# danthegoodman1/ObjectKV

Measured on AMD Instinct MI355X. Metric: GiB/s device-resident SST block decode + M rows/s, at 1/2/4/8 MI355X, higher is better.
Workload: dtype u8; 1 GPU; C3: 65536 x 64 KiB blocks, Zipf key 8-256 B / value 0-4096 B, full decode (arenas + SoA); blocks_per_gpu=65536, segment_bytes_per_gpu=4300412312, block_bytes_per_gpu=4294967296, original_bytes_per_gpu=3848907004, rows_per_gpu=1837903, mode=full, parallelism=1 independent segments (no collective)

## Files before the change

### __graft_entry__.py

```python
from __future__ import annotations

import os
import subprocess
import sys

ROOT = os.path.dirname(os.path.abspath(__file__))


def build() -> None:
    env = dict(os.environ, PYTORCH_ROCM_ARCH="gfx950")
    subprocess.run(["make", "-s", "-C", os.path.join(ROOT, "objectkv_amd", "csrc")], check=True,
                   env=env)
    subprocess.run(["make", "-s", "-C", os.path.join(ROOT, "oracle")], check=True)
    if ROOT not in sys.path:
        sys.path.insert(0, ROOT)
    import objectkv_amd
    objectkv_amd.lib()


def smoke() -> None:
    if ROOT not in sys.path:
        sys.path.insert(0, ROOT)
    import numpy as np

    import objectkv_amd as okv
    from oracle import coracle

    for kind, seed, th, bs in ((okv.sst.SYNTH_ZIPF, 3, 57344, 65536),
                               (okv.sst.SYNTH_FIXED, 1, 3584, 4096)):
        w = okv.synth_segment(kind, seed, nblocks=16, threshold=th, block_size=bs)
        seg, descs = w.data(), w.descs()[:16]
        dec = okv.Decoder(0)
        got = dec.decode(seg, descs)
        ref = coracle.decode_soa(seg, coracle.descs_array([tuple(int(x) for x in d)
                                                           for d in descs]))
# ... 29 lines not shown
```

### objectkv_amd/csrc/okv_ctx.hpp

```cpp
#pragma once
#include <hip/hip_runtime.h>

#include <algorithm>
#include <cstdlib>
#include <string>
#include <vector>

#include "okv_kernels.hpp"
#include "okv_sst.h"

namespace okv {
struct EncScratch;
void enc_release(okv_ctx* ctx);
namespace mrg {
struct Scratch;
}
void merge_release(okv_ctx* ctx);
void launch_hash(hipStream_t stream, const uint8_t* seg, uint64_t seg_bytes, const Desc* descs,
                 uint32_t nblk, uint64_t* out);
void launch_zstd_cap(hipStream_t s, const Desc* descs, uint32_t nblk, uint64_t* cap_off);
int zstd_run(okv_ctx* ctx, const uint8_t* seg, uint64_t seg_bytes, const Desc* descs,
             uint32_t nblk, uint64_t* total);
void launch_zstd_desc(hipStream_t s, const Desc* descs, uint32_t nblk, const uint64_t* cap_off,
                      const uint64_t* dec_len, Desc* out);
constexpr uint32_t kZstdLitBytes = 1u << 17;
}

struct okv_ctx {
  int device = 0;
  hipStream_t stream = nullptr;
// ... 7 lines not shown
  uint32_t* d_big = nullptr;
  uint32_t* d_ctr = nullptr;
  uint32_t big_slot = 0;
  size_t cap_blocks = 0;
  bool fused = true;
  uint32_t fused_max = 0;
  bool zstd_one_pass = false;
  bool point = true;
  uint32_t* f_flag = nullptr;
  okv::Prefix* f_agg = nullptr;
  okv::Prefix* f_incl = nullptr;
  unsigned long long* f_ctr = nullptr;
  unsigned long long f_base = 0;
  uint32_t f_epoch = 0;
  bool group = false;
  uint32_t* g_flag = nullptr;
  okv::Prefix* g_agg = nullptr;
  okv::Prefix* g_incl = nullptr;
  size_t g_cap = 0;
  uint32_t g_epoch = 0;
  uint32_t last_path = 0;
  okv_ctx* chain = nullptr;
  std::vector<okv_ctx*> chained_by;
  hipEvent_t p3_done = nullptr;
  bool p3_rec = false;
  size_t f_cap = 0;
  okv::Totals* d_tot = nullptr;
  okv::Totals* h_tot = nullptr;
  unsigned long long* d_span = nullptr;
  unsigned long long* h_span = nullptr;
  okv::SpanHint span_hint;
  bool pieces = false;
  bool stream_lb = false;
  uint64_t small_piece = 0;
  void* d_ptot = nullptr;
  hipStream_t stream2 = nullptr;
  hipEvent_t ev_piece[2] = {nullptr, nullptr};
  okv::Totals* d_tot2 = nullptr;
  uint8_t* d_seg = nullptr;
  size_t cap_seg = 0;
  okv::Desc* d_desc = nullptr;
  size_t cap_desc = 0;
  void* d_out = nullptr;
  size_t cap_out = 0;
  uint64_t* d_hash = nullptr;
  size_t cap_hash = 0;
// ... 95 lines not shown
```

### objectkv_amd/csrc/okv_decode.hip

```cpp
#include <hip/hip_runtime.h>

#include <algorithm>
#include <atomic>
#include <cstdio>
#include <cstdlib>
#include <cstring>
#include <string>
#include <vector>

#include "okv_ctx.hpp"
#include "okv_kernels.hpp"
#include "okv_sst.h"

namespace okv {

__device__ __forceinline__ uint64_t rec_index(uint32_t , uint32_t b, uint32_t r) {
  return uint64_t(b) * kRCap + r;
}
constexpr uint32_t kRecChunk = 16;

__global__ __launch_bounds__(kThreads) void okv_count_kernel(
    const uint8_t* __restrict__ seg, uint64_t seg_bytes, const Desc* __restrict__ descs,
    uint32_t nblk, int comp, BlockCount* __restrict__ cnt, Prefix* __restrict__ lp,
    Prefix* __restrict__ tile_tot, uint32_t* __restrict__ rt_pos, uint16_t* __restrict__ rt_kl,
// ... 5 lines not shown
  __shared__ uint32_t s_pos[kThreads * (kRecChunk + 1)];
  __shared__ __align__(16) uint16_t s_kl[kThreads * kRecChunk];
  __shared__ uint32_t s_rows[kThreads];
  const uint32_t tid = threadIdx.x;
  const uint32_t b = blockIdx.x * kTile + tid;
  uint64_t rows = 0, kb = 0, vb = 0, p = 0;
  int32_t st = OKV_BLK_OK;
  if (blockIdx.x == 0 && tid == 0 && big_zero) *big_zero = 0;
  uint64_t len = 0, orig = 0, off = 0;
  bool walking = false;
  if (b < nblk) {
    const Desc d = descs[b];
    const int32_t pre = pre_status ? pre_status[b] : int32_t(OKV_BLK_OK);
    if (pre != OKV_BLK_OK) {
      st = pre;
    } else if ((st = go_read_status(d, seg_bytes)) != OKV_BLK_OK) {
    } else if (comp == OKV_COMP_ZSTD) {
      st = OKV_BLK_UNSUPPORTED;
    } else {
      len = (comp == OKV_COMP_LZ4) ? 0 : d.block_size;
      orig = go_walk_bound(d.original_size);
      off = d.offset;
      walking = true;
      if (prefetch && orig && len) {
        const uint64_t first = off & ~uint64_t(3);
        const uint64_t last = (off + (orig < len ? orig : len) - 1) & ~uint64_t(3);
        uint32_t v[32];
#pragma unroll
        for (int u = 0; u < 32; ++u) {
          uint64_t a = (off & ~uint64_t(127)) + 128ull * u;
          a = a < first ? first : (a > last ? last : a);
          v[u] = *reinterpret_cast<const uint32_t*>(seg + a);
        }
        uint32_t acc = 0;
#pragma unroll
        for (int u = 0; u < 32; ++u) acc ^= v[u];
        asm volatile("" ::"v"(acc));
      }
    }
  }
  const uint32_t b0 = blockIdx.x * kTile;
  for (uint32_t c = 0; c < uint32_t(kRCap) / kRecChunk; ++c) {
    const uint64_t cap = uint64_t(c + 1) * kRecChunk;
    if (walking) {
      while (p < orig && rows < cap) {
        if (len - p < 6) { st = OKV_BLK_PANIC; break; }
        uint32_t kl, vl;
        header_global(seg, off + p, kl, vl);
        const uint64_t room = len - p - 6;
        if (kl > room || vl > room - kl) {
          st = OKV_BLK_PANIC;
          break;
        }
        const uint32_t slot = uint32_t(rows) & (kRecChunk - 1);
        s_pos[tid * (kRecChunk + 1) + slot] = uint32_t(p);
        s_kl[tid * kRecChunk + slot] = uint16_t(kl);
        rows++;
        kb += kl;
        vb += vl;
        p += 6 + uint64_t(kl) + uint64_t(vl);
      }
      if (st != OKV_BLK_OK) walking = false;
    }
    s_rows[tid] = st == OKV_BLK_OK ? uint32_t(rows) : 0u;
    __syncthreads();
    for (uint32_t q = tid; q < uint32_t(kTile) * 4; q += kThreads) {
      const uint32_t lb = q >> 2, sub = q & 3, slot = c * kRecChunk + sub * 4;
      if (b0 + lb < nblk && slot < s_rows[lb]) {
        const uint32_t* s = &s_pos[lb * (kRecChunk + 1) + sub * 4];
        *reinterpret_cast<uint4*>(rt_pos + rec_index(nblk, b0 + lb, slot)) =
            make_uint4(s[0], s[1], s[2], s[3]);
// ... 147 lines not shown
  const BlockCount* cnt;
  const Prefix* lp;
  const Prefix* tile_pre;
  const uint32_t* rt_pos;
  const uint16_t* rt_kl;
  uint32_t* big_list;
  uint32_t* big_count;
  uint64_t* row_start;
  uint64_t* key_base;
  uint64_t* val_base;
  int32_t* blk_status;
  uint64_t* key_off;
  uint16_t* key_len;
  uint64_t* val_off;
  uint32_t* val_len;
  uint8_t* key_arena;
  uint8_t* val_arena;
  uint64_t row_cap, key_cap, val_cap;
  uint64_t* vsrc;
  uint32_t* vtile;
  uint4* bchunk;
  const Totals* tot;
  uint64_t span_cap;
};

constexpr uint32_t kSwTile = 4096;
__device__ __forceinline__ bool sweep_safe(const Totals& T, uint32_t nbig, uint64_t row_cap,
                                           uint64_t key_cap, uint64_t val_cap) {
  return nbig == 0 && T.rows <= row_cap && T.kb <= key_cap && T.vb <= val_cap;
}

struct BlockBase {
  uint64_t row0, kb0, vb0;
  int32_t st;
};
__device__ __forceinline__ BlockBase block_base_of(const CopyParams& P, const BlockCount& c,
                                                   const Prefix& l, const Prefix& t) {
  BlockBase r;
  r.row0 = t.rows + l.rows;
  r.kb0 = t.kb + l.kb;
  r.vb0 = t.vb + l.vb;
  r.st = c.status;
  if (r.st == OKV_BLK_OK &&
      (r.row0 + c.rows > P.row_cap ||
       (!P.index_only && (r.kb0 + round16(c.kbytes) > P.key_cap ||
                          r.vb0 + round16(c.vbytes) > P.val_cap))))
// ... 213 lines not shown
    default:
      return make_uint4(funnel(y.x, x.w, r), funnel(y.y, y.x, r), funnel(y.z, y.y, r),
                        funnel(y.w, y.z, r));
  }
}

__device__ __noinline__ uint4 tile_chunk_pieces(const uint8_t* seg, uint64_t seg_bytes, uint64_t off,
                                                const uint32_t* pre, const uint32_t* sb,
                                                uint32_t rows, uint32_t r, uint32_t x,
                                                uint32_t lo, uint32_t hi) {
  const uint32_t dend = min(hi, pre[rows]);
  uint4 out = make_uint4(0, 0, 0, 0);
  for (uint32_t d = lo; d < dend; ++r) {
    const uint32_t e = min(dend, pre[r + 1]);
    if (e > d) {
      out = merge_bytes(out, window16(seg, seg_bytes, int64_t(off + sb[r] + x)), int32_t(d - x),
                        int32_t(e - x));
      d = e;
    }
  }
  return out;
}

template <uint32_t kT, uint32_t kNT, bool kXcd, uint32_t kSkip = 0>
__device__ __forceinline__ void tile_pass(const CopyParams& P, uint32_t tpb, uint32_t ntile) {
  constexpr uint32_t kG = kT / 64 + 8;
  constexpr bool kSector = (kSkip & 128) != 0;
  constexpr bool kLineCut = !(kSkip & 64) && !kSector;
  constexpr bool kKeyRound = kSector && !(kSkip & 256);
  constexpr uint32_t kLineExt = (kLineCut || (kSkip & 512)) ? 512 : 0;
  __shared__ TileRows<kT> R;
  __shared__ uint8_t gt[1][kG];
  __shared__ uint4 stage[(kT + kLineExt) / 16 + 4];
  uint32_t L = blockIdx.x;
  if constexpr (kXcd) L = (blockIdx.x & 7u) * (gridDim.x >> 3) + (blockIdx.x >> 3);
  if (L >= ntile) return;
  const uint32_t b = __builtin_amdgcn_readfirstlane(L / tpb);
  const uint32_t t = L - b * tpb;
  const uint32_t tid = threadIdx.x, lane = tid & 63;
  uint32_t rec = 0, kl = 0;
  if (tid < 64) {
    rec = P.rt_pos[rec_index(P.nblk, b, lane)];
    kl = P.rt_kl[rec_index(P.nblk, b, lane)];
  }
  const uint64_t off = P.descs[b].offset;
  const BlockCount c = P.cnt[b];
  const Prefix lpre = P.lp[b], tpre = P.tile_pre[b / kTile];
  asm volatile("" ::"s"(off), "s"(c.rows), "s"(c.kbytes), "s"(c.vbytes), "s"(c.pend),
               "s"(c.status), "s"(lpre.rows), "s"(lpre.kb), "s"(lpre.vb), "s"(tpre.rows),
               "s"(tpre.kb), "s"(tpre.vb));
  const uint64_t row0 = tpre.rows + lpre.rows, kb0 = tpre.kb + lpre.kb, vb0 = tpre.vb + lpre.vb;
  const bool fits = row0 + c.rows <= P.row_cap &&
                    (P.index_only ||
                     (kb0 + round16(c.kbytes) <= P.key_cap && vb0 + round16(c.vbytes) <= P.val_cap));
  const int32_t st = (c.status == OKV_BLK_OK && !fits) ? int32_t(OKV_BLK_CAPACITY) : c.status;
  auto block_outputs = [&]() {
    if (t == 0 && tid == 0) {
      P.row_start[b] = row0;
      if (P.key_base) P.key_base[b] = kb0;
      if (P.val_base) P.val_base[b] = vb0;
      P.blk_status[b] = st;
    }
  };
  const uint64_t pend = c.pend;
  const uint32_t P0 = t * kT;
  if (st != OKV_BLK_OK || c.rows == 0 || c.rows > uint64_t(kRCap) || pend > P.span_cap ||
      pend >= (uint64_t(1) << 32) || P0 >= pend) {
    block_outputs();
    return;
  }
  const uint32_t rows = uint32_t(c.rows), lastr = rows - 1;
  const uint32_t P1 = uint32_t(min<uint64_t>(uint64_t(P0) + kT, pend));
  const bool last_tile = P1 == pend;
  const int64_t A = int64_t((off + P0) & ~uint64_t(15)) - 16;
  const int64_t E = int64_t((off + P1 + 15) & ~uint64_t(15)) + 16 + (last_tile ? 0 : kLineExt);
  const uint32_t np = uint32_t((E - A) >> 4);
  if (!P.index_only && tid >= 64) {
    const int64_t lim = int64_t(round16(P.seg_bytes));
    const uint32_t u = tid - 64;
    for (uint32_t k0 = 0; k0 < np; k0 += kNT - 64) {
      const uint32_t i = k0 + u;
      if (i < np) {
        int64_t a = A + (int64_t(i) << 4);
        if (a < 0 || a + 16 > lim) a = int64_t(off) & ~int64_t(15);
        __builtin_amdgcn_global_load_lds(P.seg + a, OKV_LDS_PTR(stage + k0 + (u & ~63u)), 16,
                                         0, 0);
      }
    }
  }
  if (tid < 64) {
// ... 140 lines not shown
        const bool eb = piece && (e & 15);
        const uint64_t m = __ballot(eb);
        const uint32_t head = (X2 < X3 && (X2 & 15)) ? 1u : 0u;
        const uint32_t idx = head + uint32_t(__builtin_amdgcn_mbcnt_hi(
                                        uint32_t(m >> 32), __builtin_amdgcn_mbcnt_lo(uint32_t(m), 0u)));
        if (eb) R.bnd[idx] = ((e >> 4) << 8) | lane;
        const uint32_t nunit = __builtin_amdgcn_readlane(ui, 63);
        if (lane == 0) {
          if (head) R.bnd[0] = ((X2 >> 4) << 8) | jv;
          R.nbnd = head + uint32_t(__builtin_popcountll(m));
          R.nunit = nunit;
        }
      }
    }
    if (P.index_only && t == 0 && live) {
      const uint64_t g = row0 + lane;
      P.key_len[g] = uint16_t(k);
      P.val_len[g] = v;
      P.key_off[g] = off + ks;
      P.val_off[g] = off + vs;
    }
  }
  if (P.index_only) {
    block_outputs();
    return;
  }
  if (tid >= 64) asm volatile("s_waitcnt vmcnt(0)" ::: "memory");
  __syncthreads();
  if (t == 0 && tid < 64) {
    block_outputs();
    if (!(kSkip & 1) && lane < rows) {
      const uint64_t g = row0 + lane;
      const uint32_t kp = R.pre[0][lane], vp = R.pre[1][lane];
      P.key_len[g] = uint16_t(R.pre[0][lane + 1] - kp);
      P.val_len[g] = R.pre[1][lane + 1] - vp;
      P.key_off[g] = kb0 + kp;
      P.val_off[g] = vb0 + vp;
    }
  }
  const uint32_t kx0 = R.x[0], kx1 = R.x[1], vx0 = R.x[2], vx1 = R.x[3];
  const uint32_t nk = kx1 > kx0 ? ((kx1 + 15) >> 4) - (kx0 >> 4) : 0u;
  const uint32_t sbias = uint32_t(int64_t(off) - A);
  {
    const uint32_t nunit = R.nunit, nbnd = R.nbnd;
    uint8_t* const varena = P.val_arena + vb0;
    for (uint32_t u = tid >> 6; u < ((kSkip & 2) ? 0u : nunit); u += kNT / 64) {
      const uint32_t c0 = __builtin_amdgcn_readfirstlane(R.unit[0][u]);
      const uint32_t sbyte = __builtin_amdgcn_readfirstlane(R.unit[1][u]);
      const uint32_t cnt = __builtin_amdgcn_readfirstlane(R.unit[2][u]);
      if (lane < cnt) {
        const uint32_t line = (sbyte >> 4) + lane;
// ... 1159 lines not shown
  if ((rc = grow(ctx, reinterpret_cast<void**>(&ctx->z_dec), &ctx->z_cap_dec, total + 64)))
    return rc;
  if ((rc = zstd_run(ctx, d_seg, seg_bytes, d_desc, nblk, &total))) return rc;
  launch_zstd_desc(ctx->stream, d_desc, nblk, ctx->z_cap_off, ctx->z_dec_len, ctx->z_desc);
  OKV_HIP(hipGetLastError());
  *w = Work{ctx->z_dec, total + 16, ctx->z_desc, OKV_COMP_NONE, ctx->z_status};
  return OKV_OK;
}

uint32_t gather_threads(const okv_ctx* ctx, const Work& w, uint32_t nblk) {
  if (ctx->gather_threads) return ctx->gather_threads;
  return nblk && w.seg_bytes / nblk <= 16384 ? 64u : 256u;
}

int launch_plan(okv_ctx* ctx, const Work& w, uint32_t nblk, uint64_t* d_row_start,
                bool timed = false, uint16_t* rt_kl = nullptr, uint64_t span_cap = ~0ull,
                unsigned long long* span_max = nullptr) {
  int rc = ensure_blocks(ctx, nblk);
  if (rc) return rc;
  const uint32_t ntiles = std::max<uint32_t>(1, (nblk + kTile - 1) / kTile);
  int prefetch = nblk && w.seg_bytes <= (64ull << 20) && w.seg_bytes / nblk <= 16384;
#ifdef OKV_ABLATE
  if (const char* v = getenv("OKV_COUNT_PREFETCH")) prefetch = atoi(v) && nblk;
#endif
  hipLaunchKernelGGL(okv_count_kernel, dim3(ntiles), dim3(kThreads), 0, ctx->stream, w.seg,
                     w.seg_bytes, w.descs, nblk, w.comp, ctx->d_cnt, ctx->d_lp, ctx->d_tile_tot,
                     ctx->d_rec, rt_kl, ctx->d_big, big_counter(ctx), w.pre, prefetch, span_cap,
                     ctx->d_tile_pre, ctx->d_tot, d_row_start, ctx->d_ctr + kCtrArrive,
                     big_counter(ctx, 1), nullptr, 0u, span_max);
  OKV_HIP(hipGetLastError());
  ctx->big_slot ^= 1u;
  if (timed) prof_mark(ctx, 2);
  return OKV_OK;
}

struct TileGeo {
  uint32_t tpb;
  uint64_t span_cap;
};
TileGeo tile_geo(const okv_ctx* ctx, const Work& w, uint32_t nblk, bool index_only) {
  if (index_only || !nblk) return {1, ~0ull};
  const uint64_t kT = uint64_t(ctx->tile_kib) << 10;
  uint64_t span = (w.seg_bytes / nblk) & ~uint64_t(4095);
  if (span < 4096) span = 4096;
  const SpanHint& h = ctx->span_hint;
  if (h.nblk == nblk && h.seg == w.seg && h.descs == w.descs && h.seg_bytes == w.seg_bytes)
    span = std::max<uint64_t>(span, (h.span + 4095) & ~uint64_t(4095));
  uint64_t tpb = std::min<uint64_t>(64, (span + kT - 1) / kT);
  while (tpb > 1 && uint64_t(nblk) * tpb >= (uint64_t(1) << 31)) tpb >>= 1;
  return {uint32_t(tpb), tpb * kT};
}

template <uint32_t kT, uint32_t kNT, bool kXcd, int kDiag>
void launch_tile_t(hipStream_t s, const CopyParams& P, uint32_t tpb, uint32_t ntile) {
  const uint32_t grid = kXcd ? ((ntile + 7u) & ~7u) : ntile;
#ifdef OKV_ABLATE
  if constexpr (kDiag == 9) {
    hipLaunchKernelGGL((okv_tile_kernel_w7<kT, kNT, kXcd>), dim3(grid), dim3(kNT), 0, s, P, tpb,
                       ntile);
    return;
  } else if constexpr (kDiag >= 32) {
    hipLaunchKernelGGL((okv_tile_kernel_skip<kT, kNT, kXcd, uint32_t(kDiag - 32)>), dim3(grid),
                       dim3(kNT), 0, s, P, tpb, ntile);
  } else {
    hipLaunchKernelGGL((okv_tile_kernel_diag<kT, kNT, kXcd, kDiag>), dim3(grid), dim3(kNT), 0, s,
                       P, tpb, ntile);
  }
#else
  static_assert(kDiag == 0, "the product library has no diagnostic arms");
  hipLaunchKernelGGL((okv_tile_kernel<kT, kNT, kXcd>), dim3(grid), dim3(kNT), 0, s, P, tpb, ntile);
#endif
}
typedef void (*TileLaunch)(hipStream_t, const CopyParams&, uint32_t, uint32_t);
struct TileForm {
  uint32_t kib, threads, diag;
  TileLaunch x, plain;
};
#define OKV_TILE_FORM(K, N, D)                                                              \
  TileForm {                                                                                \
    K, N, D, launch_tile_t<K * 1024, N, true, D>, launch_tile_t<K * 1024, N, false, D>      \
  }
#ifdef OKV_ABLATE
const TileForm kTileForms[] = {OKV_TILE_FORM(16, 256, 0), OKV_TILE_FORM(8, 256, 0),
                               OKV_TILE_FORM(32, 256, 0), OKV_TILE_FORM(16, 512, 0),
                               OKV_TILE_FORM(32, 512, 0), OKV_TILE_FORM(4, 256, 0),
                               OKV_TILE_FORM(16, 256, 1), OKV_TILE_FORM(16, 256, 2),
                               OKV_TILE_FORM(16, 256, 3), OKV_TILE_FORM(16, 256, 4),
                               OKV_TILE_FORM(16, 256, 5), OKV_TILE_FORM(16, 256, 6),
                               OKV_TILE_FORM(16, 256, 7), OKV_TILE_FORM(16, 256, 8),
                               OKV_TILE_FORM(8, 256, 8), OKV_TILE_FORM(32, 512, 8),
                               OKV_TILE_FORM(16, 256, 9), OKV_TILE_FORM(64, 1024, 0),
                               OKV_TILE_FORM(64, 512, 0),
                               OKV_TILE_FORM(16, 256, 32), OKV_TILE_FORM(16, 256, 33),
                               OKV_TILE_FORM(16, 256, 34), OKV_TILE_FORM(16, 256, 36),
                               OKV_TILE_FORM(16, 256, 40), OKV_TILE_FORM(16, 256, 48),
                               OKV_TILE_FORM(16, 256, 63),
                               OKV_TILE_FORM(16, 256, 96),
                               OKV_TILE_FORM(16, 256, 160), OKV_TILE_FORM(16, 256, 672),
                               OKV_TILE_FORM(16, 256, 928)};
const TileForm* tile_form(uint32_t kib, uint32_t threads, uint32_t diag) {
  for (const TileForm& f : kTileForms)
    if (f.kib == kib && f.threads == threads && f.diag == diag) return &f;
  return nullptr;
}
#endif
void launch_tile(okv_ctx* ctx, const CopyParams& P, const TileGeo& g) {
#ifdef OKV_ABLATE
  const TileForm* f = tile_form(ctx->tile_kib, ctx->tile_threads, ctx->tile_diag);
  (ctx->tile_xcd ? f->x : f->plain)(ctx->stream, P, g.tpb, P.nblk * g.tpb);
#else
  launch_tile_t<16384, 256, true, 0>(ctx->stream, P, g.tpb, P.nblk * g.tpb);
#endif
}

int read_totals(okv_ctx* ctx, Totals* out) {
  OKV_HIP(hipMemcpyAsync(ctx->h_tot, ctx->d_tot, sizeof(Totals), hipMemcpyDeviceToHost,
                         ctx->stream));
  OKV_HIP(hipStreamSynchronize(ctx->stream));
  *out = *ctx->h_tot;
  return OKV_OK;
}

int ensure_fused(okv_ctx* ctx, uint32_t nblk) {
  const size_t n = std::max<size_t>(nblk, 1);
  if (n <= ctx->f_cap && ctx->f_flag) return OKV_OK;
  if (ctx->f_flag) {
    OKV_HIP(hipStreamSynchronize(ctx->stream));
    (void)hipFree(ctx->f_flag);
    (void)hipFree(ctx->f_agg);
    (void)hipFree(ctx->f_incl);
  }
  OKV_HIP(hipMalloc(&ctx->f_flag, n * sizeof(uint64_t)));
  OKV_HIP(hipMemsetAsync(ctx->f_flag, 0, n * sizeof(uint64_t), ctx->stream));
  OKV_HIP(hipMalloc(&ctx->f_agg, n * sizeof(Prefix)));
  OKV_HIP(hipMalloc(&ctx->f_incl, n * sizeof(Prefix)));
  if (!ctx->f_ctr) {
    OKV_HIP(hipMalloc(&ctx->f_ctr, 2 * sizeof(unsigned long long)));
    OKV_HIP(hipMemsetAsync(ctx->f_ctr, 0, 2 * sizeof(unsigned long long), ctx->stream));
    ctx->f_base = 0;
  }
  ctx->f_cap = n;
  return OKV_OK;
}

#ifdef OKV_ABLATE
#include "okv_decode_ablate_host.inc"
#endif

int decode_device(okv_ctx* ctx, const uint8_t* seg, uint64_t seg_bytes, const Desc* descs,
                  uint32_t nblk, int comp, okv_decode_out* o, uint32_t flags) {
  const bool index_only = flags & OKV_F_INDEX_ONLY;
  if (!o->row_start || !o->blk_status) return set_err(ctx, OKV_E_ARG, "row_start/blk_status");
  if (!aligned16(seg)) return set_err(ctx, OKV_E_ARG, "device seg must be 16-byte aligned");
  if (!index_only && (!aligned16(o->key_arena) || !aligned16(o->val_arena)))
    return set_err(ctx, OKV_E_ARG, "device arenas must be 16-byte aligned");
  prof_mark(ctx, 0);
  Work w;
  int rc = prepare(ctx, seg, seg_bytes, descs, nblk, comp, index_only, &w);
  if (rc) return rc;
  prof_mark(ctx, 1);
  const bool fused =
      ctx->fused && nblk && nblk <= ctx->fused_max && gather_threads(ctx, w, nblk) == 64;
#ifdef OKV_ABLATE
  const bool stream = ctx->stream_lb && ctx->fused && nblk > ctx->fused_max &&
                      gather_threads(ctx, w, nblk) == 64;
#else
  constexpr bool stream = false;
#endif
  const bool large = nblk && !fused && !stream && gather_threads(ctx, w, nblk) == 256;
#ifdef OKV_ABLATE
// ... 69 lines not shown
  P.span_cap = geo.span_cap;
  P.big_list = ctx->d_big;
  P.big_count = big_count;
  P.cnt = ctx->d_cnt;
  P.lp = ctx->d_lp;
  P.tile_pre = ctx->d_tile_pre;
  P.row_start = o->row_start;
  P.key_base = o->key_base;
  P.val_base = o->val_base;
  P.blk_status = o->blk_status;
  P.key_off = o->key_off;
  P.key_len = o->key_len;
  P.val_off = o->val_off;
  P.val_len = o->val_len;
  P.key_arena = o->key_arena;
  P.val_arena = o->val_arena;
  P.row_cap = o->row_cap;
  P.key_cap = index_only ? 0 : o->key_cap;
  P.val_cap = index_only ? 0 : o->val_cap;
  P.vsrc = nullptr;
  P.vtile = nullptr;
  P.bchunk = nullptr;
  P.tot = ctx->d_tot;
  uint64_t sw_tiles = 0;
  if (sweep) {
    sw_tiles = (o->val_cap + kSwTile - 1) / kSwTile;
    if ((rc = grow(ctx, &ctx->d_vsrc, &ctx->cap_vsrc, std::max<uint64_t>(o->row_cap, 1) * 24 + 256)) ||
        (rc = grow(ctx, &ctx->d_vtile, &ctx->cap_vtile, (sw_tiles + 4) * 4)))
      return rc;
    P.vsrc = static_cast<uint64_t*>(ctx->d_vsrc);
    P.bchunk = reinterpret_cast<uint4*>(static_cast<uint8_t*>(ctx->d_vsrc) +
                                        ((std::max<uint64_t>(o->row_cap, 1) * 8 + 255) & ~255ull));
    P.vtile = static_cast<uint32_t*>(ctx->d_vtile);
  }
  const uint32_t gt = nblk ? gather_threads(ctx, w, nblk) : 0;
  ctx->last_path = (comp ? OKV_PATH_ZSTD : 0u) |
                   (comp == OKV_COMP_ZSTD && !index_only && ctx->z_retried ? OKV_PATH_ZSTD_REGROW : 0u) |
                   (!nblk ? 0u
                    : fused ? OKV_PATH_FUSED
                    : stream ? OKV_PATH_STREAM
                    : group ? OKV_PATH_GROUP | OKV_PATH_BIG
                    : OKV_PATH_BIG | (tile ? OKV_PATH_TILE
                                      : sweep ? OKV_PATH_SWEEP | OKV_PATH_STAGED
                                      : gt == 256 && ctx->gather_staged && !index_only
                                          ? OKV_PATH_STAGED
                                      : gt == 64 && ctx->gather_staged ? OKV_PATH_SMALL
                                                                       : OKV_PATH_GATHER));
  const uint32_t nbig_grid = std::min<uint32_t>(nblk, 512);
  auto launch_big = [&]() {
    if (index_only)
      hipLaunchKernelGGL(okv_index_kernel, dim3((nbig_grid + kThreads - 1) / kThreads),
                         dim3(kThreads), 0, ctx->stream, P);
    else
      hipLaunchKernelGGL(okv_copy_kernel, dim3(nbig_grid), dim3(kThreads), 0, ctx->stream, P);
  };
  if (early_big) {
    launch_big();
    OKV_HIP(hipGetLastError());
    prof_mark(ctx, 3);
  }
  if (ctx->chain && ctx->chain->p3_rec)
    OKV_HIP(hipStreamWaitEvent(ctx->stream, ctx->chain->p3_done, 0));
  if (nblk) {
    const dim3 g(ctx->gather_grid ? std::min<uint32_t>(nblk, ctx->gather_grid) : nblk);
#ifdef OKV_ABLATE
    if (block_diag) {
      hipLaunchKernelGGL((okv_block_kernel<1024, false>), dim3(nblk), dim3(1024), 0, ctx->stream, P,
                         FusedParams{});
    } else
#endif
    if (fused || stream || block) {
      FusedParams F;
      F.pre = w.pre;
      F.cnt = ctx->d_cnt;
      F.lp = ctx->d_lp;
      F.tile_pre = ctx->d_tile_pre;
      F.flag = ctx->f_flag;
      F.agg = ctx->f_agg;
      F.incl = ctx->f_incl;
      F.ctr = ctx->f_ctr;
      F.arr = ctx->f_ctr + 1;
      F.base = ctx->f_base;
      ctx->f_epoch = (ctx->f_epoch + 1) & 0x3fffffffu;
      F.epoch = ctx->f_epoch;
      F.tot = ctx->d_tot;
// ... 24 lines not shown
      G.tile_pre = ctx->d_tile_pre;
      G.flag = ctx->g_flag;
      G.agg = ctx->g_agg;
      G.incl = ctx->g_incl;
      ctx->g_epoch = (ctx->g_epoch + 1) & 0x3fffffffu;
      if (!ctx->g_epoch) ctx->g_epoch = 1;
      G.epoch = ctx->g_epoch;
      G.tot = ctx->d_tot;
      G.big_zero = big_counter(ctx, 1);
      hipLaunchKernelGGL(okv_group_kernel, dim3((nblk + kGroup - 1) / kGroup), dim3(kThreads), 0,
                         ctx->stream, P, G);
      OKV_HIP(hipGetLastError());
      ctx->big_slot ^= 1u;
    }
#endif
    else if (tile) {
      if ((ctx->tile_diag >= 3 && ctx->tile_diag <= 5) || ctx->tile_diag == 7) {
        const size_t n = (size_t(nblk) * geo.tpb / 256 + 1) * 64;
        if ((rc = grow(ctx, &ctx->d_vsrc, &ctx->cap_vsrc, n))) return rc;
        P.vsrc = static_cast<uint64_t*>(ctx->d_vsrc);
      }
#ifdef OKV_ABLATE
      if (b0) {
        launch_tile(ctx, piece_params(P, 0, b0), geo);
        OKV_HIP(hipStreamWaitEvent(ctx->stream, ctx->ev_piece[1], 0));
        launch_tile(ctx, piece_params(P, b0, nblk - b0), geo);
      } else
#endif
        launch_tile(ctx, P, geo);
    }
#ifdef OKV_ABLATE
    else if (sweep) {
      hipLaunchKernelGGL(okv_rows_kernel, g, dim3(64), 0, ctx->stream, P);
      if (sw_tiles) {
        SweepParams S{w.seg, w.seg_bytes, o->val_off, o->val_len, P.vsrc, P.vtile, P.bchunk,
                      o->val_arena,
                      ctx->d_tot, P.big_count, o->row_cap, o->key_cap, o->val_cap};
        if (ctx->value_sweep == 5)
          hipLaunchKernelGGL((okv_value_sweep_kernel<4, true>), dim3(uint32_t((sw_tiles + 3) / 4)),
                             dim3(256), 0, ctx->stream, S);
        else if (ctx->value_sweep == 7)
          hipLaunchKernelGGL((okv_value_sweep_kernel<3, true>), dim3(uint32_t((sw_tiles + 2) / 3)),
                             dim3(256), 0, ctx->stream, S);
        else if (ctx->value_sweep == 6)
          hipLaunchKernelGGL((okv_value_sweep_kernel<2, true>), dim3(uint32_t((sw_tiles + 1) / 2)),
                             dim3(256), 0, ctx->stream, S);
        else if (ctx->value_sweep == 4)
// ... 18 lines not shown
        Totals* tot = p0 + n == nblk ? ctx->d_tot : pt + (k & 1);
        launch_count_piece(ctx, w, p0, n, o->row_start, base, tot, k == 0);
        hipLaunchKernelGGL(okv_gather_small_kernel, dim3(n), dim3(64), 0, ctx->stream,
                           piece_params(P, p0, n));
        base = tot;
      }
      ctx->big_slot ^= 1u;
    } else if (gather_threads(ctx, w, nblk) == 64 && ctx->gather_staged)
      hipLaunchKernelGGL(okv_gather_small_kernel, g, dim3(64), 0, ctx->stream, P);
    else if (gather_threads(ctx, w, nblk) == 64)
      hipLaunchKernelGGL(okv_gather_kernel<64>, g, dim3(64), 0, ctx->stream, P);
    else
      hipLaunchKernelGGL(okv_gather_kernel<kThreads>, g, dim3(kThreads), 0, ctx->stream, P);
#else
    else if (gather_threads(ctx, w, nblk) == 64) {
      hipLaunchKernelGGL(okv_gather_small_kernel, g, dim3(64), 0, ctx->stream, P);
    } else {
      return set_err(ctx, OKV_E_ARG, "decode path");
    }
#endif
    if (!block && !early_big) launch_big();
    OKV_HIP(hipGetLastError());
  }
  if (ctx->p3_done) {
    OKV_HIP(hipEventRecord(ctx->p3_done, ctx->stream));
    ctx->p3_rec = true;
  }
  prof_mark(ctx, 4);
  if (flags & OKV_F_ASYNC) return OKV_OK;
  Totals T;
  rc = read_totals(ctx, &T);
  if (rc) return rc;
  o->n_rows = T.rows;
  o->key_bytes = index_only ? 0 : T.kb;
  o->val_bytes = index_only ? 0 : T.vb;
  o->n_bad_blocks = T.bad;
  if (T.rows > o->row_cap || (!index_only && (T.kb > o->key_cap || T.vb > o->val_cap)))
    return set_err(ctx, OKV_E_CAPACITY, "output capacity too small (totals set)");
  return OKV_OK;
}

bool output_bounds(const uint8_t* , uint64_t seg_bytes, const okv_block_desc* descs,
                   uint32_t nblk, int comp, uint64_t limit, uint64_t* rows, uint64_t* bytes) {
  if (comp == OKV_COMP_ZSTD) return false;
  uint64_t r = 0, by = 0;
  for (uint32_t b = 0; b < nblk; ++b) {
// ... 296 lines not shown
  okv_ctx* ctx = okv_open_on_stream(device, stream);
  if (ctx && opts) {
    if (opts->flags & OKV_OPEN_NO_FUSED) ctx->fused = false;
    ctx->zstd_one_pass = (opts->flags & OKV_OPEN_ZSTD_ONE_PASS) != 0;
    ctx->point = (opts->flags & OKV_OPEN_NO_POINT) == 0;
  }
  return ctx;
}

okv_ctx* okv_open_on_stream(int device, void* stream) {
  int n = 0;
  if (hipGetDeviceCount(&n) != hipSuccess || device < 0 || device >= n) return nullptr;
  if (hipSetDevice(device) != hipSuccess) return nullptr;
  okv_ctx* ctx = new okv_ctx();
  ctx->device = device;
  {
    int ncu = 0, per_cu = 0;
    if (hipDeviceGetAttribute(&ncu, hipDeviceAttributeMultiprocessorCount, device) != hipSuccess ||
        hipOccupancyMaxActiveBlocksPerMultiprocessor(&per_cu, okv_decode_fused_kernel, 64, 0) !=
            hipSuccess)
      ncu = per_cu = 0;
    ctx->fused_max = std::min<uint32_t>(kFusedMaxBlocks, uint32_t(ncu) * uint32_t(per_cu) / 4);
    if (ctx->fused_max == 0) ctx->fused = false;
  }
#ifdef OKV_ABLATE
  if (const char* v = getenv("OKV_GATHER_THREADS")) {
    ctx->gather_threads = uint32_t(atoi(v));
    if (ctx->gather_threads != 64 && ctx->gather_threads != 256) {
      delete ctx;
      return nullptr;
    }
  }
  if (const char* v = getenv("OKV_GATHER_GRID")) ctx->gather_grid = uint32_t(atoi(v));
  if (const char* v = getenv("OKV_DECODE_FUSED")) ctx->fused = atoi(v) != 0;
  if (const char* v = getenv("OKV_DECODE_GROUP")) ctx->group = atoi(v) != 0;
  if (const char* v = getenv("OKV_DECODE_PIECES")) ctx->pieces = atoi(v) != 0;
  if (const char* v = getenv("OKV_DECODE_STREAM")) ctx->stream_lb = atoi(v) != 0;
  if (const char* v = getenv("OKV_SMALL_PIECE_MB")) ctx->small_piece = uint64_t(atoi(v)) << 20;
  if (const char* v = getenv("OKV_GATHER_STAGED")) ctx->gather_staged = atoi(v) != 0;
  if (const char* v = getenv("OKV_VALUE_SWEEP")) {
    ctx->value_sweep = uint32_t(atoi(v));
    if (ctx->value_sweep > 11 || ctx->value_sweep == 3) {
      delete ctx;
      return nullptr;
    }
  }
  if (const char* v = getenv("OKV_TILE")) {
    ctx->tile_kib = uint32_t(atoi(v));
// ... 28 lines not shown
  return ctx;
}

okv_ctx* okv_open(int device) { return okv_open_on_stream(device, nullptr); }

void okv_close(okv_ctx* ctx) {
  if (!ctx) return;
  (void)hipSetDevice(ctx->device);
  if (ctx->stream) (void)hipStreamSynchronize(ctx->stream);
  for (okv_ctx* c : ctx->chained_by)
    if (c->chain == ctx) c->chain = nullptr;
  if (ctx->chain) {
    auto& v = ctx->chain->chained_by;
    v.erase(std::remove(v.begin(), v.end(), ctx), v.end());
  }
  (void)hipFree(ctx->d_cnt);
  (void)hipFree(ctx->d_lp);
  (void)hipFree(ctx->d_tile_tot);
  (void)hipFree(ctx->d_tile_pre);
  (void)hipFree(ctx->d_rec);
  (void)hipFree(ctx->d_big);
  (void)hipFree(ctx->d_ctr);
  if (ctx->p3_done) (void)hipEventDestroy(ctx->p3_done);
  (void)hipFree(ctx->f_flag);
  (void)hipFree(ctx->f_agg);
  (void)hipFree(ctx->f_incl);
  (void)hipFree(ctx->g_flag);
  (void)hipFree(ctx->g_agg);
  (void)hipFree(ctx->g_incl);
  (void)hipFree(ctx->f_ctr);
  (void)hipFree(ctx->d_tot);
  if (ctx->h_tot) (void)hipHostFree(ctx->h_tot);
  if (ctx->h_span) (void)hipHostFree(ctx->h_span);
  (void)hipFree(ctx->d_span);
  (void)hipFree(ctx->d_seg);
  (void)hipFree(ctx->d_desc);
  (void)hipFree(ctx->d_out);
  (void)hipFree(ctx->d_hash);
  if (ctx->h_slab) (void)hipHostFree(ctx->h_slab);
  (void)hipFree(ctx->d_vsrc);
  (void)hipFree(ctx->d_hdr);
  (void)hipFree(ctx->d_vtile);
  (void)hipFree(ctx->z_cap_off);
  (void)hipFree(ctx->z_dec_len);
  (void)hipFree(ctx->z_status);
  (void)hipFree(ctx->z_desc);
// ... 10 lines not shown
  (void)hipFree(ctx->z_need);
  if (ctx->stream2) {
    (void)hipStreamSynchronize(ctx->stream2);
    (void)hipStreamDestroy(ctx->stream2);
  }
  for (hipEvent_t& ev : ctx->ev_piece)
    if (ev) (void)hipEventDestroy(ev);
  (void)hipFree(ctx->d_tot2);
  okv::enc_release(ctx);
  okv::merge_release(ctx);
  if (ctx->own_stream && ctx->stream) (void)hipStreamDestroy(ctx->stream);
  delete ctx;
}

const char* okv_last_error(const okv_ctx* ctx) { return ctx ? ctx->err.c_str() : "no context"; }
void* okv_stream(const okv_ctx* ctx) { return ctx ? ctx->stream : nullptr; }

int okv_decode_chain(okv_ctx* ctx, okv_ctx* after) {
  if (!ctx || after == ctx || (after && after->device != ctx->device))
    return set_err(ctx, OKV_E_ARG, "okv_decode_chain: contexts");
  int prev = -1;
  OKV_HIP(hipGetDevice(&prev));
  for (okv_ctx* c : {ctx, after}) {
    if (c && !c->p3_done) {
      OKV_HIP(hipSetDevice(c->device));
      const hipError_t e = hipEventCreateWithFlags(&c->p3_done, hipEventDisableTiming);
      if (e != hipSuccess) {
        (void)hipSetDevice(prev);
        return set_err(ctx, OKV_E_HIP, "okv_decode_chain: event", e);
      }
    }
  }
  OKV_HIP(hipSetDevice(prev));
  if (ctx->chain) {
    auto& v = ctx->chain->chained_by;
    v.erase(std::remove(v.begin(), v.end(), ctx), v.end());
  }
  ctx->chain = after;
  if (after) after->chained_by.push_back(ctx);
  return OKV_OK;
}

int okv_sync(okv_ctx* ctx) {
  if (!ctx) return OKV_E_ARG;
  OKV_HIP(hipStreamSynchronize(ctx->stream));
  return OKV_OK;
}

// ... 186 lines not shown
```

### objectkv_amd/csrc/okv_decode_ablate.inc

```
template <int NT>
__global__ __launch_bounds__(NT) void okv_gather_kernel(CopyParams P) {
  __shared__ GatherSmem sm;
  for (uint32_t b = blockIdx.x; b < P.nblk; b += gridDim.x) {
    const BlockMeta m = block_meta(P, b);
    if (block_head(P, b, m)) {
      const int rows = int(m.c.rows);
      const GlobalWin src{P.seg, P.seg_bytes, m.off};
      if (threadIdx.x < 64) {
        const uint32_t t = threadIdx.x;
        const uint32_t rec = int(t) < rows ? P.rt_pos[rec_index(P.nblk, b, t)] : 0u;
        build_row_table(src, sm, rows, rec);
      }
      __syncthreads();
      write_row_index(P, sm, m, rows);
      if (!P.index_only) {
        gather_region<false>(src, sm, rows, P.key_arena, m.B.kb0, threadIdx.x >> 6, NT / 64);
        gather_region<true>(src, sm, rows, P.val_arena, m.B.vb0, threadIdx.x >> 6, NT / 64);
      }
    }
    if (b + gridDim.x < P.nblk) __syncthreads();
  }
}

__global__ __launch_bounds__(64) void okv_rows_kernel(CopyParams P) {
// ... 340 lines not shown
  const BlockCount c = P.cnt[b];
  const Prefix lpre = P.lp[b], tpre = P.tile_pre[b / kTile];
  asm volatile("" ::"s"(off), "s"(c.rows), "s"(c.kbytes), "s"(c.vbytes), "s"(c.pend),
               "s"(c.status), "s"(lpre.rows), "s"(lpre.kb), "s"(lpre.vb), "s"(tpre.rows),
               "s"(tpre.kb), "s"(tpre.vb));
  if constexpr (kProbe) T[1] = __builtin_amdgcn_s_memrealtime();
  const uint64_t row0 = tpre.rows + lpre.rows, kb0 = tpre.kb + lpre.kb, vb0 = tpre.vb + lpre.vb;
  const bool fits = row0 + c.rows <= P.row_cap &&
                    (P.index_only ||
                     (kb0 + round16(c.kbytes) <= P.key_cap && vb0 + round16(c.vbytes) <= P.val_cap));
  const int32_t st = (c.status == OKV_BLK_OK && !fits) ? int32_t(OKV_BLK_CAPACITY) : c.status;
  auto block_outputs = [&]() {
    if (t == 0 && tid == 0) {
      P.row_start[b] = row0;
      if (P.key_base) P.key_base[b] = kb0;
      if (P.val_base) P.val_base[b] = vb0;
      P.blk_status[b] = st;
    }
  };
  const uint64_t pend = c.pend;
  const uint32_t P0 = t * kT;
  if (st != OKV_BLK_OK || c.rows == 0 || c.rows > uint64_t(kRCap) || pend > P.span_cap ||
      pend >= (uint64_t(1) << 32) || P0 >= pend) {
    block_outputs();
    return;
  }
  const uint32_t rows = uint32_t(c.rows), lastr = rows - 1;
  const uint32_t P1 = uint32_t(min<uint64_t>(uint64_t(P0) + kT, pend));
  const bool last_tile = P1 == pend;
  const int64_t A = int64_t((off + P0) & ~uint64_t(15)) - 16;
  const int64_t E = int64_t((off + P1 + 15) & ~uint64_t(15)) + 16;
  const uint32_t np = uint32_t((E - A) >> 4);
  if (!P.index_only && kDiag != 2 && !kDirect && tid >= 64) {
    const int64_t lim = int64_t(round16(P.seg_bytes));
    const uint32_t u = tid - 64;
    for (uint32_t k0 = 0; k0 < np; k0 += kNT - 64) {
      const uint32_t i = k0 + u;
      if (i < np) {
        int64_t a = A + (int64_t(i) << 4);
        if (a < 0 || a + 16 > lim) a = int64_t(off) & ~int64_t(15);
        __builtin_amdgcn_global_load_lds(P.seg + a, OKV_LDS_PTR(stage + k0 + (u & ~63u)), 16,
                                         0, 0);
      }
    }
  }
  if constexpr (kProbe) T[2] = __builtin_amdgcn_s_memrealtime();
// ... 72 lines not shown
        const uint64_t m = __ballot(eb);
        const uint32_t head = (X2 < X3 && (X2 & 15)) ? 1u : 0u;
        const uint32_t idx = head + uint32_t(__builtin_amdgcn_mbcnt_hi(
                                        uint32_t(m >> 32), __builtin_amdgcn_mbcnt_lo(uint32_t(m), 0u)));
        if (eb) R.bnd[idx] = ((e >> 4) << 8) | lane;
        const uint32_t nunit = __builtin_amdgcn_readlane(ui, 63);
        if (lane == 0) {
          if (head) R.bnd[0] = ((X2 >> 4) << 8) | jv;
          R.nbnd = head + uint32_t(__builtin_popcountll(m));
          R.nunit = nunit;
        }
      }
    }
    if (P.index_only && t == 0 && live) {
      const uint64_t g = row0 + lane;
      P.key_len[g] = uint16_t(k);
      P.val_len[g] = v;
      P.key_off[g] = off + ks;
      P.val_off[g] = off + vs;
    }
  }
  if constexpr (kProbe) T[3] = __builtin_amdgcn_s_memrealtime();
  if (P.index_only) {
    block_outputs();
    return;
  }
  if (tid >= 64) asm volatile("s_waitcnt vmcnt(0)" ::: "memory");
  __syncthreads();
  if constexpr (kProbe) T[4] = __builtin_amdgcn_s_memrealtime();
  if (t == 0 && tid < 64) {
    block_outputs();
    if (lane < rows) {
      const uint64_t g = row0 + lane;
      const uint32_t kp = R.pre[0][lane], vp = R.pre[1][lane];
      P.key_len[g] = uint16_t(R.pre[0][lane + 1] - kp);
      P.val_len[g] = R.pre[1][lane + 1] - vp;
      P.key_off[g] = kb0 + kp;
      P.val_off[g] = vb0 + vp;
    }
  }
  const uint32_t kx0 = R.x[0], kx1 = R.x[1], vx0 = R.x[2], vx1 = R.x[3];
  const uint32_t nk = kx1 > kx0 ? ((kx1 + 15) >> 4) - (kx0 >> 4) : 0u;
  const uint32_t nv = vx1 > vx0 ? ((vx1 + 15) >> 4) - (vx0 >> 4) : 0u;
  const uint32_t sbias = uint32_t(int64_t(off) - A);
  if (kDiag == 1) return;
  if constexpr (kRuns) {
    const uint32_t nunit = R.nunit, nbnd = R.nbnd;
    uint8_t* const varena = P.val_arena + vb0;
    for (uint32_t u = tid >> 6; u < nunit; u += kNT / 64) {
      const uint32_t c0 = __builtin_amdgcn_readfirstlane(R.unit[0][u]);
      const uint32_t sbyte = __builtin_amdgcn_readfirstlane(R.unit[1][u]);
// ... 145 lines not shown
```

### objectkv_amd/csrc/okv_kernels.hpp

```cpp
#pragma once
#include <hip/hip_runtime.h>
#include <stdint.h>

#include "okv_sst.h"

namespace okv {

constexpr int kThreads = 256;
constexpr int kTile = 256;
constexpr int kRowBatch = 256;
constexpr int kFastRows = 1024;
constexpr int kRCap = 64;
constexpr int kStage = 65536;
constexpr int kStagePad = 64;

struct BlockCount {
  uint64_t rows;
  uint64_t kbytes;
  uint64_t vbytes;
  uint64_t pend;
  int32_t status;
  int32_t pad;
};

// ... 17 lines not shown
  uint64_t span = 0;
};

__host__ __device__ inline uint64_t round16(uint64_t x) { return (x + 15) & ~uint64_t(15); }

constexpr uint64_t kGoMaxAlloc = uint64_t(1) << 48;
__host__ __device__ inline uint64_t go_walk_bound(uint64_t original_size) {
  return int64_t(original_size) < 0 ? 0 : original_size;
}
__host__ __device__ inline int32_t go_read_status(const Desc& d, uint64_t seg_bytes) {
  if (int64_t(d.offset) < 0) return OKV_BLK_EOF;
  if (d.block_size > kGoMaxAlloc) return OKV_BLK_PANIC;
  if (d.offset >= seg_bytes) return OKV_BLK_EOF;
  if (seg_bytes - d.offset < d.block_size) return OKV_BLK_SHORT;
  return OKV_BLK_OK;
}

#define OKV_LDS_PTR(p) ((__attribute__((address_space(3))) void*)(p))

__device__ __forceinline__ uint32_t funnel(uint32_t hi, uint32_t lo, uint32_t sh) {
  return __builtin_amdgcn_alignbyte(hi, lo, sh);
}

__device__ __forceinline__ void header_global(const uint8_t* __restrict__ seg, uint64_t pos,
                                              uint32_t& klen, uint32_t& vlen) {
  const uint32_t* w = reinterpret_cast<const uint32_t*>(seg + (pos & ~uint64_t(3)));
  const uint32_t sh = uint32_t(pos & 3);
  const uint32_t w0 = w[0];
  const uint32_t w1 = w[1];
  const uint32_t w2 = (sh == 3) ? w[2] : 0u;
  const uint32_t a = funnel(w1, w0, sh);
  const uint32_t b = funnel(w2, w1, sh);
  klen = a & 0xffffu;
  vlen = (a >> 16) | (b << 16);
}

__device__ __forceinline__ void header_lds(const uint32_t* sw, uint32_t bi, uint32_t& klen,
                                           uint32_t& vlen) {
  const uint32_t* w = sw + (bi >> 2);
  const uint32_t sh = bi & 3;
  const uint32_t a = funnel(w[1], w[0], sh);
  const uint32_t b = funnel(w[2], w[1], sh);
  klen = a & 0xffffu;
  vlen = (a >> 16) | (b << 16);
}

__device__ __forceinline__ uint4 load16_lds(const uint32_t* sw, uint32_t bi) {
  const uint32_t* w = sw + (bi >> 2);
  const uint32_t sh = bi & 3;
  const uint32_t w0 = w[0], w1 = w[1], w2 = w[2], w3 = w[3], w4 = w[4];
  return make_uint4(funnel(w1, w0, sh), funnel(w2, w1, sh), funnel(w3, w2, sh),
                    funnel(w4, w3, sh));
}
// ... 154 lines not shown
```

Before: 2931 GiB/s.

## Hand off chained decodes via in-kernel release word instead of stream events

Adds an optional chain handoff in which one tile-kernel block, chosen a configurable lead before the end of the grid, atomically writes an epoch to signal memory. A chained context waits on that value with hipStreamWaitValue64 instead of waiting for the whole previous decode's completion event, so the next decode can start while the tail of the previous one drains. A host backstop write keeps the epoch sequence correct, and an optional nontemporal header-read variant is added to the count kernel for chained runs. The build now targets the ablate configuration, which changes the default compiled path, and the benchmark runs a single unchained GPU, so the handoff is probably not exercised.

```diff
diff --git a/__graft_entry__.py b/__graft_entry__.py
--- a/__graft_entry__.py
+++ b/__graft_entry__.py
@@ -9,8 +9,8 @@
 
 def build() -> None:
     env = dict(os.environ, PYTORCH_ROCM_ARCH="gfx950")
-    subprocess.run(["make", "-s", "-C", os.path.join(ROOT, "objectkv_amd", "csrc")], check=True,
-                   env=env)
+    subprocess.run(["make", "-s", "-j4", "-C", os.path.join(ROOT, "objectkv_amd", "csrc"),
+                    "ablate"], check=True, env=env)
     subprocess.run(["make", "-s", "-C", os.path.join(ROOT, "oracle")], check=True)
     if ROOT not in sys.path:
         sys.path.insert(0, ROOT)
diff --git a/objectkv_amd/csrc/okv_chain.hpp b/objectkv_amd/csrc/okv_chain.hpp
--- /dev/null
+++ b/objectkv_amd/csrc/okv_chain.hpp
@@ -0,0 +1,32 @@
+#pragma once
+#include <cstdint>
+
+namespace okv {
+
+struct ChainEpochs {
+  static constexpr uint64_t kMax = (uint64_t(1) << 63) - 1;
+  uint64_t taken = 0;
+  uint64_t enqueued = 0;
+  uint64_t take() {
+    if (taken < kMax) ++taken;
+    return taken;
+  }
+  void wrote(uint64_t e) {
+    if (e > enqueued) enqueued = e;
+  }
+  uint64_t told() const { return enqueued; }
+};
+
+inline uint32_t release_index(uint32_t grid, uint32_t ntile, uint32_t lead, bool xcd) {
+  uint32_t i = grid > lead ? grid - lead : 0u;
+  auto tile = [&](uint32_t x) { return xcd ? (x & 7u) * (grid >> 3) + (x >> 3) : x; };
+  while (i && tile(i) >= ntile) --i;
+  return i;
+}
+
+inline uint32_t release_lead(uint32_t resident, uint32_t pct) {
+  const uint64_t l = uint64_t(resident) * pct / 100;
+  return l < 1 ? 1u : l > 0xffffffffull ? 0xffffffffu : uint32_t(l);
+}
+
+}
diff --git a/objectkv_amd/csrc/okv_ctx.hpp b/objectkv_amd/csrc/okv_ctx.hpp
--- a/objectkv_amd/csrc/okv_ctx.hpp
+++ b/objectkv_amd/csrc/okv_ctx.hpp
@@ -6,6 +6,7 @@
 #include <string>
 #include <vector>
 
+#include "okv_chain.hpp"
 #include "okv_kernels.hpp"
 #include "okv_sst.h"
 
@@ -59,6 +60,13 @@
   uint32_t last_path = 0;
   okv_ctx* chain = nullptr;
   std::vector<okv_ctx*> chained_by;
+  bool chain_word = false;
+  unsigned long long* rel_word = nullptr;
+  okv::ChainEpochs rel;
+  uint32_t tile_resident = 0;
+  uint32_t rel_lead = 1;
+  bool chain_nt = false;
+  std::vector<okv_ctx*> rel_waiters, rel_waited;
   hipEvent_t p3_done = nullptr;
   bool p3_rec = false;
   size_t f_cap = 0;
diff --git a/objectkv_amd/csrc/okv_decode.hip b/objectkv_amd/csrc/okv_decode.hip
--- a/objectkv_amd/csrc/okv_decode.hip
+++ b/objectkv_amd/csrc/okv_decode.hip
@@ -51,7 +51,7 @@
       orig = go_walk_bound(d.original_size);
       off = d.offset;
       walking = true;
-      if (prefetch && orig && len) {
+      if ((prefetch & 1) && orig && len) {
         const uint64_t first = off & ~uint64_t(3);
         const uint64_t last = (off + (orig < len ? orig : len) - 1) & ~uint64_t(3);
         uint32_t v[32];
@@ -75,7 +75,12 @@
       while (p < orig && rows < cap) {
         if (len - p < 6) { st = OKV_BLK_PANIC; break; }
         uint32_t kl, vl;
-        header_global(seg, off + p, kl, vl);
+#if defined(OKV_ABLATE) || defined(OKV_CHAIN_NT)
+        if (prefetch & 2)
+          header_global<true>(seg, off + p, kl, vl);
+        else
+#endif
+          header_global(seg, off + p, kl, vl);
         const uint64_t room = len - p - 6;
         if (kl > room || vl > room - kl) {
           st = OKV_BLK_PANIC;
@@ -269,6 +274,9 @@
   uint4* bchunk;
   const Totals* tot;
   uint64_t span_cap;
+  unsigned long long* rel_word;
+  unsigned long long rel_epoch;
+  uint32_t rel_idx;
 };
 
 constexpr uint32_t kSwTile = 4096;
@@ -528,6 +536,18 @@
   return out;
 }
 
+#if defined(OKV_ABLATE) || defined(OKV_CHAIN_WORD)
+#define OKV_CHAIN_HAS_WORD 1
+#endif
+__device__ __forceinline__ void chain_release(const CopyParams& P) {
+#ifdef OKV_CHAIN_HAS_WORD
+  if (P.rel_word && blockIdx.x == P.rel_idx && threadIdx.x == 0)
+    __hip_atomic_store(P.rel_word, P.rel_epoch, __ATOMIC_RELAXED, __HIP_MEMORY_SCOPE_SYSTEM);
+#else
+  (void)P;
+#endif
+}
+
 template <uint32_t kT, uint32_t kNT, bool kXcd, uint32_t kSkip = 0>
 __device__ __forceinline__ void tile_pass(const CopyParams& P, uint32_t tpb, uint32_t ntile) {
   constexpr uint32_t kG = kT / 64 + 8;
@@ -572,6 +592,7 @@
   const uint32_t P0 = t * kT;
   if (st != OKV_BLK_OK || c.rows == 0 || c.rows > uint64_t(kRCap) || pend > P.span_cap ||
       pend >= (uint64_t(1) << 32) || P0 >= pend) {
+    chain_release(P);
     block_outputs();
     return;
   }
@@ -758,11 +779,13 @@
     }
   }
   if (P.index_only) {
+    chain_release(P);
     block_outputs();
     return;
   }
   if (tid >= 64) asm volatile("s_waitcnt vmcnt(0)" ::: "memory");
   __syncthreads();
+  chain_release(P);
   if (t == 0 && tid < 64) {
     block_outputs();
     if (!(kSkip & 1) && lane < rows) {
@@ -1968,6 +1991,10 @@
   int prefetch = nblk && w.seg_bytes <= (64ull << 20) && w.seg_bytes / nblk <= 16384;
 #ifdef OKV_ABLATE
   if (const char* v = getenv("OKV_COUNT_PREFETCH")) prefetch = atoi(v) && nblk;
+  if (ctx->chain && ctx->chain_nt) prefetch |= 2;
+#endif
+#ifdef OKV_CHAIN_NT
+  if (ctx->chain) prefetch |= 2;
 #endif
   hipLaunchKernelGGL(okv_count_kernel, dim3(ntiles), dim3(kThreads), 0, ctx->stream, w.seg,
                      w.seg_bytes, w.descs, nblk, w.comp, ctx->d_cnt, ctx->d_lp, ctx->d_tile_tot,
@@ -1998,8 +2025,11 @@
 }
 
 template <uint32_t kT, uint32_t kNT, bool kXcd, int kDiag>
-void launch_tile_t(hipStream_t s, const CopyParams& P, uint32_t tpb, uint32_t ntile) {
+void launch_tile_t(hipStream_t s, const CopyParams& P0, uint32_t tpb, uint32_t ntile,
+                   uint32_t lead) {
   const uint32_t grid = kXcd ? ((ntile + 7u) & ~7u) : ntile;
+  CopyParams P = P0;
+  P.rel_idx = release_index(grid, ntile, lead, kXcd);
 #ifdef OKV_ABLATE
   if constexpr (kDiag == 9) {
     hipLaunchKernelGGL((okv_tile_kernel_w7<kT, kNT, kXcd>), dim3(grid), dim3(kNT), 0, s, P, tpb,
@@ -2017,7 +2047,7 @@
   hipLaunchKernelGGL((okv_tile_kernel<kT, kNT, kXcd>), dim3(grid), dim3(kNT), 0, s, P, tpb, ntile);
 #endif
 }
-typedef void (*TileLaunch)(hipStream_t, const CopyParams&, uint32_t, uint32_t);
+typedef void (*TileLaunch)(hipStream_t, const CopyParams&, uint32_t, uint32_t, uint32_t);
 struct TileForm {
   uint32_t kib, threads, diag;
   TileLaunch x, plain;
@@ -2050,12 +2080,16 @@
   return nullptr;
 }
 #endif
+#ifndef OKV_CHAIN_LEAD_PCT
+#define OKV_CHAIN_LEAD_PCT 50
+#endif
+constexpr uint32_t kChainLeadPct = OKV_CHAIN_LEAD_PCT;
 void launch_tile(okv_ctx* ctx, const CopyParams& P, const TileGeo& g) {
 #ifdef OKV_ABLATE
   const TileForm* f = tile_form(ctx->tile_kib, ctx->tile_threads, ctx->tile_diag);
-  (ctx->tile_xcd ? f->x : f->plain)(ctx->stream, P, g.tpb, P.nblk * g.tpb);
+  (ctx->tile_xcd ? f->x : f->plain)(ctx->stream, P, g.tpb, P.nblk * g.tpb, ctx->rel_lead);
 #else
-  launch_tile_t<16384, 256, true, 0>(ctx->stream, P, g.tpb, P.nblk * g.tpb);
+  launch_tile_t<16384, 256, true, 0>(ctx->stream, P, g.tpb, P.nblk * g.tpb, ctx->rel_lead);
 #endif
 }
 
@@ -2092,6 +2126,55 @@
 #ifdef OKV_ABLATE
 #include "okv_decode_ablate_host.inc"
 #endif
+
+struct ChainBackstop {
+  okv_ctx* ctx;
+  uint64_t e;
+  hipError_t enqueue() {
+    const hipError_t r = hipStreamWriteValue64(ctx->stream, ctx->rel_word, e, 0);
+    if (r == hipSuccess) ctx->rel.wrote(e);
+    e = 0;
+    return r;
+  }
+  int write() {
+    if (e) OKV_HIP(enqueue());
+    return OKV_OK;
+  }
+  ~ChainBackstop() {
+    if (e) (void)enqueue();
+  }
+};
+
+void chain_note_wait(okv_ctx* ctx, okv_ctx* a) {
+  auto add = [](std::vector<okv_ctx*>& v, okv_ctx* c) {
+    if (std::find(v.begin(), v.end(), c) == v.end()) v.push_back(c);
+  };
+  add(a->rel_waiters, ctx);
+  add(ctx->rel_waited, a);
+}
+
+bool chain_word_alloc(okv_ctx* c) {
+  if (!c->chain_word) return false;
+  int can = 0;
+  if (hipDeviceGetAttribute(&can, hipDeviceAttributeCanUseStreamWaitValue, c->device) !=
+          hipSuccess ||
+      !can)
+    return false;
+  void* p = nullptr;
+  if (hipExtMallocWithFlags(&p, sizeof(unsigned long long), hipMallocSignalMemory) != hipSuccess ||
+      !p) {
+    (void)hipGetLastError();
+    return false;
+  }
+  if (hipStreamWriteValue64(c->stream, p, 0, 0) != hipSuccess) {
+    (void)hipGetLastError();
+    (void)hipFree(p);
+    return false;
+  }
+  c->rel_word = static_cast<unsigned long long*>(p);
+  c->rel = ChainEpochs{};
+  return true;
+}
 
 int decode_device(okv_ctx* ctx, const uint8_t* seg, uint64_t seg_bytes, const Desc* descs,
                   uint32_t nblk, int comp, okv_decode_out* o, uint32_t flags) {
@@ -2207,6 +2290,9 @@
   P.vtile = nullptr;
   P.bchunk = nullptr;
   P.tot = ctx->d_tot;
+  P.rel_word = nullptr;
+  P.rel_epoch = 0;
+  P.rel_idx = 0;
   uint64_t sw_tiles = 0;
   if (sweep) {
     sw_tiles = (o->val_cap + kSwTile - 1) / kSwTile;
@@ -2244,8 +2330,21 @@
     OKV_HIP(hipGetLastError());
     prof_mark(ctx, 3);
   }
-  if (ctx->chain && ctx->chain->p3_rec)
-    OKV_HIP(hipStreamWaitEvent(ctx->stream, ctx->chain->p3_done, 0));
+  if (okv_ctx* const a = ctx->chain) {
+    if (a->rel_word) {
+      if (const uint64_t e = a->rel.told()) {
+        OKV_HIP(hipStreamWaitValue64(ctx->stream, a->rel_word, e, hipStreamWaitValueGte,
+                                     ~uint64_t(0)));
+        chain_note_wait(ctx, a);
+      }
+    } else if (a->p3_rec) {
+      OKV_HIP(hipStreamWaitEvent(ctx->stream, a->p3_done, 0));
+    }
+  }
+  ChainBackstop backstop{ctx, ctx->rel_word ? ctx->rel.take() : 0};
+  P.rel_word = ctx->rel_word;
+  P.rel_epoch = backstop.e;
+  P.rel_idx = 0;
   if (nblk) {
     const dim3 g(ctx->gather_grid ? std::min<uint32_t>(nblk, ctx->gather_grid) : nblk);
 #ifdef OKV_ABLATE
@@ -2316,7 +2415,9 @@
       }
 #ifdef OKV_ABLATE
       if (b0) {
-        launch_tile(ctx, piece_params(P, 0, b0), geo);
+        CopyParams first = piece_params(P, 0, b0);
+        first.rel_word = nullptr;
+        launch_tile(ctx, first, geo);
         OKV_HIP(hipStreamWaitEvent(ctx->stream, ctx->ev_piece[1], 0));
         launch_tile(ctx, piece_params(P, b0, nblk - b0), geo);
       } else
@@ -2381,6 +2482,7 @@
     if (!block && !early_big) launch_big();
     OKV_HIP(hipGetLastError());
   }
+  if ((rc = backstop.write())) return rc;
   if (ctx->p3_done) {
     OKV_HIP(hipEventRecord(ctx->p3_done, ctx->stream));
     ctx->p3_rec = true;
@@ -2723,8 +2825,21 @@
       ncu = per_cu = 0;
     ctx->fused_max = std::min<uint32_t>(kFusedMaxBlocks, uint32_t(ncu) * uint32_t(per_cu) / 4);
     if (ctx->fused_max == 0) ctx->fused = false;
-  }
+    int tile_per_cu = 0;
+    if (hipOccupancyMaxActiveBlocksPerMultiprocessor(
+            &tile_per_cu, okv_tile_kernel<16384, 256, true>, 256, 0) != hipSuccess)
+      tile_per_cu = 0;
+    ctx->tile_resident = uint32_t(ncu) * uint32_t(std::max(tile_per_cu, 0));
+    ctx->rel_lead = release_lead(ctx->tile_resident, kChainLeadPct);
+  }
+#ifdef OKV_CHAIN_WORD
+  ctx->chain_word = true;
+#endif
 #ifdef OKV_ABLATE
+  if (const char* v = getenv("OKV_CHAIN_LEAD_PCT"))
+    ctx->rel_lead = release_lead(ctx->tile_resident, uint32_t(atoi(v)));
+  if (const char* v = getenv("OKV_CHAIN_HANDOFF")) ctx->chain_word = !strcmp(v, "word");
+  if (const char* v = getenv("OKV_CHAIN_NT")) ctx->chain_nt = atoi(v) != 0;
   if (const char* v = getenv("OKV_GATHER_THREADS")) {
     ctx->gather_threads = uint32_t(atoi(v));
     if (ctx->gather_threads != 64 && ctx->gather_threads != 256) {
@@ -2799,6 +2914,16 @@
   (void)hipFree(ctx->d_big);
   (void)hipFree(ctx->d_ctr);
   if (ctx->p3_done) (void)hipEventDestroy(ctx->p3_done);
+  for (okv_ctx* w : ctx->rel_waiters) {
+    if (w->stream) (void)hipStreamSynchronize(w->stream);
+    auto& v = w->rel_waited;
+    v.erase(std::remove(v.begin(), v.end(), ctx), v.end());
+  }
+  for (okv_ctx* a : ctx->rel_waited) {
+    auto& v = a->rel_waiters;
+    v.erase(std::remove(v.begin(), v.end(), ctx), v.end());
+  }
+  if (ctx->rel_word) (void)hipFree(ctx->rel_word);
   (void)hipFree(ctx->f_flag);
   (void)hipFree(ctx->f_agg);
   (void)hipFree(ctx->f_incl);
@@ -2855,8 +2980,9 @@
   int prev = -1;
   OKV_HIP(hipGetDevice(&prev));
   for (okv_ctx* c : {ctx, after}) {
-    if (c && !c->p3_done) {
+    if (c && !c->p3_done && !c->rel_word) {
       OKV_HIP(hipSetDevice(c->device));
+      if (chain_word_alloc(c)) continue;
       const hipError_t e = hipEventCreateWithFlags(&c->p3_done, hipEventDisableTiming);
       if (e != hipSuccess) {
         (void)hipSetDevice(prev);
diff --git a/objectkv_amd/csrc/okv_decode_ablate.inc b/objectkv_amd/csrc/okv_decode_ablate.inc
--- a/objectkv_amd/csrc/okv_decode_ablate.inc
+++ b/objectkv_amd/csrc/okv_decode_ablate.inc
@@ -386,6 +386,7 @@
   const uint32_t P0 = t * kT;
   if (st != OKV_BLK_OK || c.rows == 0 || c.rows > uint64_t(kRCap) || pend > P.span_cap ||
       pend >= (uint64_t(1) << 32) || P0 >= pend) {
+    chain_release(P);
     block_outputs();
     return;
   }
@@ -504,11 +505,13 @@
   }
   if constexpr (kProbe) T[3] = __builtin_amdgcn_s_memrealtime();
   if (P.index_only) {
+    chain_release(P);
     block_outputs();
     return;
   }
   if (tid >= 64) asm volatile("s_waitcnt vmcnt(0)" ::: "memory");
   __syncthreads();
+  chain_release(P);
   if constexpr (kProbe) T[4] = __builtin_amdgcn_s_memrealtime();
   if (t == 0 && tid < 64) {
     block_outputs();
diff --git a/objectkv_amd/csrc/okv_kernels.hpp b/objectkv_amd/csrc/okv_kernels.hpp
--- a/objectkv_amd/csrc/okv_kernels.hpp
+++ b/objectkv_amd/csrc/okv_kernels.hpp
@@ -63,13 +63,14 @@
   return __builtin_amdgcn_alignbyte(hi, lo, sh);
 }
 
+template <bool kStream = false>
 __device__ __forceinline__ void header_global(const uint8_t* __restrict__ seg, uint64_t pos,
                                               uint32_t& klen, uint32_t& vlen) {
   const uint32_t* w = reinterpret_cast<const uint32_t*>(seg + (pos & ~uint64_t(3)));
   const uint32_t sh = uint32_t(pos & 3);
-  const uint32_t w0 = w[0];
-  const uint32_t w1 = w[1];
-  const uint32_t w2 = (sh == 3) ? w[2] : 0u;
+  const uint32_t w0 = kStream ? __builtin_nontemporal_load(w) : w[0];
+  const uint32_t w1 = kStream ? __builtin_nontemporal_load(w + 1) : w[1];
+  const uint32_t w2 = (sh == 3) ? (kStream ? __builtin_nontemporal_load(w + 2) : w[2]) : 0u;
   const uint32_t a = funnel(w1, w0, sh);
   const uint32_t b = funnel(w2, w1, sh);
   klen = a & 0xffffu;
```

Result: slower. 2892 GiB/s (-1.3%).
